# solonas13/REAL

Measured on AMD Instinct MI355X. Metric: aligned reads/sec (100 bp, k≤3) at 1/2/4/8 MI355X; achieved HBM GB/s vs peak, higher is better.
Workload: dtype u64

## Files before the change

### real_amd/csrc/match_kernel.hip

```cpp
#include "match_common.h"
#include "row_bytes.h"

#ifndef RH_ABLATE
#define RH_ABLATE 0
#endif
#ifndef RH_PHASE_TIMING
#define RH_PHASE_TIMING 0
#endif

#ifndef RH_PHASE_SUB
#define RH_PHASE_SUB 0
#endif
#if RH_PHASE_TIMING
#define PH_NOW() ((unsigned)__builtin_amdgcn_s_memrealtime())
#define PH_SUB(N, DT) do { if (RH_PHASE_SUB == (N)) s.tD += (DT); else if (RH_PHASE_SUB == 4) s.tD -= (DT); } while (0)
#else
#define PH_NOW() 0u
#endif
#define EB 8
#define MQ 16
#define QUEUE_BYTES (MQ * 64u * 5u + 6u * 64u * 4u)
enum : int { TK_STARTS = 0, TK_DIRECTORY = 1, TK_ROWS = 3, TK_ROWS_WIDE = 4 };
__host__ __device__ constexpr uint32_t stg_bytes(int W, int TK) { return TK >= TK_ROWS ? 11008u : (W <= 4 ? QUEUE_BYTES : 9728u); }
#define MQR 8u
static_assert(MQR == RH_QSPILL_SLOTS, "the spill area holds a second queue of MQR slots per lane");
#define NPEND2 24
#define MQR2 24u
#define STG_PAD 16u
#ifndef RH_KEEP_TW_MAXW
#define RH_KEEP_TW_MAXW 4
#endif
#define NPEND 4
#define SLOT_NONE 31u
#define SLOT_BIG 30u
#define PEND_OVF 0xffu
#define BIG_T 48u
#define BIG_T2 1024u

template <int W_, bool SCORES_, bool ALL_, int TK_, bool PASS2_>
struct LaneInst {
    static constexpr int W = W_;
    static constexpr bool SCORES = SCORES_;
    static constexpr bool ALL = ALL_;
    static constexpr int TK = TK_;
    static constexpr bool PASS2 = PASS2_;
    static constexpr bool DEFER = SCORES || ALL;
    static constexpr bool ROWS = TK >= TK_ROWS;
    static constexpr bool WIDE = TK == TK_ROWS_WIDE;
    static constexpr bool DIR = TK == TK_DIRECTORY;
    static constexpr bool HAS_PASS2 = ROWS && DEFER;
    static constexpr bool PAIRED = ROWS && !WIDE && DEFER && !PASS2;
    static constexpr int NP = PASS2 ? NPEND2 : NPEND;
    static constexpr uint32_t QSLOTS = PASS2 ? MQR2 : MQR;
    static constexpr uint32_t ROWBUF = QSLOTS * 64u * 5u, BKX = ROWBUF + 64u * 128u;
    static constexpr uint32_t BIG = PASS2 ? BIG_T2 : BIG_T;
    static constexpr uint32_t OVN = PASS2 ? 16u : 4u;
    static constexpr uint32_t STG = PASS2 ? BKX + 256u : stg_bytes(W, TK);
    static constexpr uint32_t STG_CAP = STG - STG_PAD - 32u;
    static_assert(!ROWS || (BKX + 256u <= STG && ROWBUF % 16 == 0), "row staging fits the wave's LDS region");
};
static_assert(QUEUE_BYTES % 16 == 0, "the staged bytes behind the queue are 16-byte aligned");

#define PM_LM_SHIFT 9
#define PM_LM_MASK (63u << PM_LM_SHIFT)
template <class T>
struct LaneState {
    static constexpr int W = T::W, NP = T::NP;
    uint64_t O[W];
    uint64_t shi, slo;
    uint32_t patl;
    int inv;
    __device__ __forceinline__ uint32_t nw() const { return (patl + 31) >> 5; }
    __device__ __forceinline__ uint64_t lastmask() const { return ~0ull << (64 - 2 * (patl - 32 * (nw() - 1))); }
    __device__ __forceinline__ uint32_t so(uint32_t l) const { return inv ? (patl - l) : 0u; }
    __device__ __forceinline__ float eps(double filter_mult) const { return (float)(filter_mult * (double)patl); }
    uint64_t r, o0, o1;
    uint64_t info;
    float iscore;
    uint32_t cpos, ck, cfrag;
    float cscore;
    bool cok;
    uint32_t crpos, ckk;
    uint32_t p_pos[NP], p_meta[NP];
    uint64_t p_tw[W <= RH_KEEP_TW_MAXW ? W : 1];
    uint32_t p_n, cslot;
    uint32_t nhit;
    unsigned cA, cB, cPw, cCw;
    __device__ __forceinline__ void addL(unsigned n) { cA += n; }
    __device__ __forceinline__ void addV(unsigned n) { cA += n << 4; }
    __device__ __forceinline__ void addS(unsigned n) { cA += n << 16; }
    __device__ __forceinline__ void addP(unsigned n) { if (T::PASS2) cPw += n; else cB += n; }
    __device__ __forceinline__ void addC(unsigned n) { if (T::PASS2) cCw += n; else cB += n << 11; }
    __device__ __forceinline__ unsigned getP() const { return T::PASS2 ? cPw : (cB & 2047u); }
    __device__ __forceinline__ unsigned getC() const { return T::PASS2 ? cCw : ((cB >> 11) & 2047u); }
    __device__ __forceinline__ void addH(unsigned n) { cB += n << 22; }
    __device__ __forceinline__ void reset_counters() { cA = cB = cPw = cCw = 0; }
    __device__ __forceinline__ void reset_read()
    {
        p_n = 0; cslot = SLOT_NONE;
#pragma unroll
        for (int j = 0; j < NP; ++j) { p_pos[j] = 0; p_meta[j] = 0; }
    }
    __device__ __forceinline__ void reset_strand(int inv_)
    {
        inv = inv_;
        cpos = 0xffffffffu; ck = 0; cfrag = 0; cscore = 1.0f; cok = false;
        crpos = 0xffffffffu; ckk = 0;
    }
#if RH_PHASE_TIMING
    unsigned tW, tD, tR;
#endif
};


template <int N>
__device__ __forceinline__ uint32_t sel(const uint32_t (&v)[N], uint32_t j)
{
    uint32_t r = 0;
#pragma unroll
    for (int i = 0; i < N; ++i) r |= j == (uint32_t)i ? v[i] : 0u;
    return r;
}
template <int N>
__device__ __forceinline__ float sel(const float (&v)[N], uint32_t j)
{
    uint32_t r = 0;
#pragma unroll
    for (int i = 0; i < N; ++i) r |= j == (uint32_t)i ? __float_as_uint(v[i]) : 0u;
    return __uint_as_float(r);
}
template <int N, class T>
__device__ __forceinline__ void put(T (&v)[N], uint32_t j, T x)
{
#pragma unroll
    for (int i = 0; i < N; ++i) v[i] = j == (uint32_t)i ? x : v[i];
}

template <class T>
__device__ __forceinline__ void deliver(const MatchArgs &a, LaneState<T> &s, uint32_t pos, uint32_t meta, float score)
{
    if (T::ALL) {
        unsigned long long slot = wave_append_slot(a.raw_count);
        if (slot < a.raw_cap) a.raw[slot] = make_uint4((uint32_t)s.r, pos, __float_as_uint(score), meta & ~PM_LM_MASK);
        s.nhit++;
    } else {
        fold_update<T::SCORES>((meta >> 8) & 1, a.t.fileid, pos, meta & 0xff, score, s.eps(a.filter_mult), meta >> 16, s.info, s.iscore);
    }
}

template <class T, class Row>
__device__ __forceinline__ void flush_pending(const MatchArgs &a, LaneState<T> &s, const double *sLL, const Row &qrow)
{
    constexpr int W = T::W, NP = T::NP;
    float sc[NP];
#pragma unroll
    for (int i = 0; i < NP; ++i) sc[i] = 1.0f;
#pragma unroll 1
    for (uint32_t j = 0; j < s.p_n; ++j) {
        if (!T::SCORES || (RH_ABLATE & 1)) break;
        const uint32_t pos = sel<NP>(s.p_pos, j);
        const uint32_t meta = sel<NP>(s.p_meta, j);
        const uint32_t inv = (meta >> 8) & 1;
        uint64_t Ow[W], tw[W];
        if ((int)inv == s.inv) {
#pragma unroll
            for (int i = 0; i < W; ++i) Ow[i] = s.O[i];
        } else {
            revcomp_words<W>(s.O, Ow, s.patl);
        }
        if (j == 0 && W <= RH_KEEP_TW_MAXW) {
#pragma unroll
            for (int i = 0; i < W; ++i) tw[i] = s.p_tw[W <= RH_KEEP_TW_MAXW ? i : 0];
        } else {
            const uint64_t wi = pos >> 5;
            const unsigned sh = 2u * (pos & 31);
            uint64_t t[W + 2];
#pragma unroll
            for (int i = 0; i <= W; i += 2) {
                U64x2 p2 = {0ull, 0ull};
                if ((uint32_t)i <= s.nw()) p2 = load2(a.t.text + wi + i);
                t[i] = p2.a; t[i + 1] = p2.b;
            }
#pragma unroll
            for (int i = 0; i < W; ++i) tw[i] = sh ? ((t[i] << sh) | (t[i + 1] >> (64 - sh))) : t[i];
        }
        const float v = score_location<W>(sLL, Ow, tw, s.patl, qrow, a.b.qual != nullptr, inv);
        put<NP>(sc, j, v);
    }
    auto lm_of = [&](uint32_t meta) { return (meta >> PM_LM_SHIFT) & 63u; };
    if (s.p_n == 1) {
        if (lm_of(s.p_meta[0])) deliver(a, s, s.p_pos[0], s.p_meta[0], sc[0]);
        return;
    }
    if (T::ALL) {
#pragma unroll 1
        for (uint32_t j = 0; j < s.p_n; ++j) {
            const uint32_t meta = sel<NP>(s.p_meta, j);
            if (lm_of(meta)) deliver(a, s, sel<NP>(s.p_pos, j), meta, sel<NP>(sc, j));
        }
        return;
    }
    if (s.p_n < 2) return;
    static_assert(NP <= 24, "two words of twelve ranks");
    uint64_t ord0 = 0, ord1 = 0;
    auto ord_at = [&](uint32_t rk) { return (uint32_t)((rk < 12 ? ord0 >> (5 * rk) : ord1 >> (5 * (rk - 12))) & 31u); };
#pragma unroll
    for (uint32_t j = 0; j < (uint32_t)NP; ++j) {
        const uint64_t kj = ((uint64_t)((s.p_meta[j] >> 8) & 1u) << 32) | s.p_pos[j];
        uint32_t rank = 0;
#pragma unroll
        for (uint32_t i = 0; i < (uint32_t)NP; ++i) {
            const uint64_t ki = ((uint64_t)((s.p_meta[i] >> 8) & 1u) << 32) | s.p_pos[i];
// ... 520 lines not shown
        }
        wave_lds_sync();
#if RH_PHASE_TIMING
        unsigned ph1 = PH_NOW();
        s.tW += ph1 - ph0;
#endif
        const bool mine = act && !(s.p_n == PEND_OVF) && !(RH_ABLATE & 8);
        const uint8_t *rowb = rowbuf + lane * 128;
        const uint32_t sw = lane & 7;
        auto row = [&](uint32_t d) { return *reinterpret_cast<const uint32_t *>(rowb + ((((d >> 2) ^ sw) << 4) | ((d & 3) << 2))); };
        uint32_t e_cnt = 0, e_j = 0, e_base = 0;
        bool e_ovf = false;
        uint32_t g, r;
        if (!wide) {
            g = rh_row_addr((uint32_t)la, sig_of(la), a.l, gbits).group;
            r = sig_of(5 - la) >> (a.l - pbits);
        } else {
            r = (uint32_t)(msig_wide(la) >> a.ix.fshift);
            g = r >> 28;
        }
        if (mine) {
            s.addL(1u);
            const uint32_t h0 = row(0), h1 = row(1);
            if (!rh_row_complex(h0, h1)) {
                e_cnt = ((g < 8 ? h0 : h1) >> (4 * (g & 7))) & 15u;
                const uint32_t m0 = g < 8 ? (g ? (h0 & (0xffffffffu >> (32 - 4 * g))) : 0u) : h0;
                const uint32_t m1 = g > 8 ? (h1 & (0xffffffffu >> (32 - 4 * (g - 8)))) : 0u;
                const uint32_t b0 = (m0 & 0x0f0f0f0fu) + ((m0 >> 4) & 0x0f0f0f0fu), b1 = (m1 & 0x0f0f0f0fu) + ((m1 >> 4) & 0x0f0f0f0fu);
                e_base = __builtin_amdgcn_sad_u8(b0, 0u, __builtin_amdgcn_sad_u8(b1, 0u, 0u));
            } else {
                e_ovf = true;
                uint32_t off = 0, sat255 = 0;
#pragma unroll
                for (int q = 0; q < 4; ++q) {
                    const uint32_t w = row(4 + q);
                    const int nb = (int)g - 4 * q;
                    const uint32_t below = nb <= 0 ? 0u : (nb >= 4 ? 0xffffffffu : ((1u << (8 * nb)) - 1u));
                    const uint32_t upto = nb < 0 ? 0u : (nb >= 3 ? 0xffffffffu : ((1u << (8 * (nb + 1))) - 1u));
                    off = __builtin_amdgcn_sad_u8(w & below, 0u, off);
                    if ((g >> 2) == (uint32_t)q) e_cnt = (w >> (8 * (g & 3))) & 255u;
                    const uint32_t y = ~w | ~upto;
                    sat255 |= (y - 0x01010101u) & ~y & 0x80808080u;
                }
                const bool sat = sat255 != 0;
                const uint32_t o0 = row(2), tot = row(3);
                e_base = o0 + off;
                if (sat) {
                    const uint2 kr = key_group_range(a.ix.ent[la], o0, o0 + tot, wide ? 28u : pbits, g);
                    e_base = kr.x; e_cnt = kr.y;
                }
            }
            if (!wide) s.addC(e_cnt);
            s.addP(e_cnt);
            if (e_cnt > T::BIG) { s.p_n = PEND_OVF; s.cslot = (!T::PASS2 && T::HAS_PASS2 && e_cnt <= BIG_T2) ? SLOT_NONE : SLOT_BIG; e_cnt = 0; }
            if (RH_ABLATE & 4) e_cnt = 0;
        }
        const uint32_t rk = wide ? rh_fp16(r) : (r >> (pbits - p16));
        U64x2 pre = {0ull, 0ull};
        if (e_ovf && e_cnt) pre = load2(reinterpret_cast<const uint64_t *>(a.ix.ent[la] + e_base));
        if (li + 1 < NL) ISSUE_ROWS(la + 1);
        auto take = [&](bool pass, uint32_t pos) {
            const bool merge = pass && qn && pos == q_last;
            if ((!wide || T::DEFER) && pass && !merge && qn >= 2) {
                for (uint32_t k = 0; k + 1 < qn; ++k)
                    if (q_pos[k * 64] == pos) { q_la[k * 64] |= (uint8_t)(1u << la); pass = false; break; }
            }
            if (pass && !merge && qn == T::QSLOTS) { s.p_n = PEND_OVF; e_cnt = 0; pass = false; }
            const uint32_t slot = merge ? qn - 1 : qn;
            const uint32_t lav = (merge ? q_lastla : 0u) | (1u << la);
            if (pass) { q_pos[slot * 64] = pos; q_la[slot * 64] = (uint8_t)lav; q_last = pos; q_lastla = lav; qn = slot + 1; }
        };
        auto passes = [&](uint32_t x) { return wide ? (x == 0u) : (__popc(((x >> 1) | x) & 0x55555555u) <= a.seedkmax); };
        uint32_t passm = 0;
        while (__any(!e_ovf && e_j < e_cnt)) {
#pragma unroll
            for (uint32_t u = 0; u < 4; ++u) {
                const uint32_t jj = e_j + u;
                const bool ok = !e_ovf && jj < e_cnt;
                const uint32_t h = ok ? rh_row_entry_hw(e_base + jj) : 4u;
                const uint32_t d0 = row(h >> 1);
                const uint32_t key = (h & 1) ? (d0 >> 16) : (d0 & 0xffffu);
                passm |= (ok && passes(key ^ rk) ? 1u : 0u) << (jj & 31u);
            }
            e_j += 4;
        }
        if (!T::PASS2 && T::HAS_PASS2 && __popc(passm) > NPEND) { s.p_n = PEND_OVF; passm = 0; e_cnt = 0; }
        while (__any(passm != 0)) {
            const bool step = passm != 0;
            const uint32_t jj = step ? (uint32_t)__ffs((int)passm) - 1u : 0u;
            passm &= passm - 1u;
            const uint32_t h = step ? rh_row_entry_hw(e_base + jj) : 4u;
            const uint32_t d0 = row(h >> 1), d1 = row((h >> 1) + 1);
            take(step, (h & 1) ? d1 : ((d0 >> 16) | (d1 << 16)));
        }
        auto take_ovf = [&](bool ok, uint2 e) { take(ok && passes(wide ? (e.x ^ r) : ((e.x & pmask) ^ r)), e.y); };
        if (__any(e_ovf && e_cnt)) {
            take_ovf(e_ovf && e_cnt > 0, make_uint2((uint32_t)pre.a, (uint32_t)(pre.a >> 32)));
            take_ovf(e_ovf && e_cnt > 1, make_uint2((uint32_t)pre.b, (uint32_t)(pre.b >> 32)));
        }
        e_j = 2;
        while (__any(e_ovf && e_j < e_cnt)) {
            uint2 e[T::OVN];
#pragma unroll
            for (uint32_t u = 0; u < T::OVN; ++u) e[u] = (e_ovf && e_j + u < e_cnt) ? a.ix.ent[la][e_base + e_j + u] : make_uint2(0u, 0u);
#pragma unroll
            for (uint32_t u = 0; u < T::OVN; ++u) take_ovf(e_ovf && e_j + u < e_cnt, e[u]);
            e_j += T::OVN;
        }
#if RH_PHASE_TIMING
        s.tD += PH_NOW() - ph1;
#endif
    }
    if (T::SCORES && qlast) ISSUE_QUALS();
#if RH_PHASE_TIMING
    const unsigned ph2 = PH_NOW();
#endif
    if (s.p_n == PEND_OVF) qn = 0;
    {
        CandText<T::W> c0;
        uint32_t rp0 = qn ? q_pos[0] : 0u;
        if (qn) cand_load(a, s, rp0, c0);
        for (uint32_t k = 0; k < qn; ++k) {
            CandText<T::W> c1;
            uint32_t rp1 = 0;
            if (k + 1 < qn) { rp1 = q_pos[(k + 1) * 64]; cand_load(a, s, rp1, c1); }
            process_loaded(a, s, sLL, rp0, (uint32_t)q_la[k * 64], c0);
            c0 = c1; rp0 = rp1;
        }
    }
#if RH_PHASE_TIMING
    s.tR += PH_NOW() - ph2;
#endif
    if (T::SCORES && qlast) ISSUE_QUALS_LATE();
#undef ISSUE_QUALS
#undef ISSUE_QUALS_LATE
#undef QUAL_DMA
}

template <class T>
__device__ __forceinline__ void match_rows_paired(const MatchArgs &a, LaneState<T> &s, const double *sLL, uint8_t *stg, bool act, uint32_t rhi,
                                                  uint32_t rlo)
{
    constexpr uint32_t QS = T::QSLOTS;
    uint32_t lane = threadIdx.x & 63;
    asm volatile("" : "+v"(lane));
    uint32_t *q_pos = reinterpret_cast<uint32_t *>(stg) + lane;
    uint8_t *q_la = stg + QS * 64 * 4 + lane;
    uint8_t *rowbuf = stg + T::ROWBUF;
    auto spill = [&](uint32_t k) -> uint2 & { return a.qspill[((size_t)(blockIdx.x * 4u + (threadIdx.x >> 6)) * QS + (k - QS)) * 64u + lane]; };
    const uint32_t bb = a.b_bits;
    const uint32_t gbits = a.ix.fbits, pbits = a.ix.pbits, p16 = pbits < 16 ? pbits : 16;
    const uint32_t pmask = (1u << pbits) - 1;
    const uint32_t mb = (1u << bb) - 1, fhi = (uint32_t)s.shi, flo = (uint32_t)s.slo;
    auto sig_of = [&](uint32_t strand, uint32_t la) {
        const uint32_t hi = strand ? rhi : fhi, lo = strand ? rlo : flo;
        const uint2 x = rh_list_segs(la);
        const uint32_t sa_ = ((x.x < 2 ? hi : lo) >> ((x.x & 1) ? 0u : bb)) & mb, sc_ = ((x.y < 2 ? hi : lo) >> ((x.y & 1) ? 0u : bb)) & mb;
        return (sa_ << bb) | sc_;
    };
    auto tbl_of = [](uint32_t li) { return li < 4 ? li >> 1 : li - 2; };
    struct Round { uint32_t row, g0, g1, s0; };
    auto round_of = [&](uint32_t li) -> Round {
        const uint32_t tbl = tbl_of(li), wbit = 1u << (gbits - 1);
        if (li < 4) {
            const RhRowAddr ra = rh_row_addr_pair(tbl, sig_of(li & 1u, tbl), a.l, gbits);
            return {ra.row, ra.group, ra.group | wbit, li & 1u};
        }
        const RhCanon c = rh_canon(sig_of(0u, tbl) >> bb, sig_of(1u, tbl) >> bb, bb);
        const RhRowAddr ra = rh_row_addr_canon(tbl, c, a.l, gbits);
        const uint32_t lo = c.self ? ra.group : ra.group & ~wbit;
        return {ra.row, lo, c.self ? lo : lo | wbit, c.which};
    };
    uint32_t qn = 0, qnf = 0, q_last = 0, q_lastla = 0;
    auto q_getp = [&](uint32_t k) { return k < QS ? q_pos[k * 64] : spill(k).x; };
    auto q_getl = [&](uint32_t k) { return k < QS ? (uint32_t)q_la[k * 64] : spill(k).y; };
    uint4 va0, va1, va2, va3, va4, va5, va6, va7;
    uint32_t *bkx = reinterpret_cast<uint32_t *>(stg + T::BKX);
#define ISSUE_ROWS_P(LI)                                                                                                    \
    do {                                                                                                                    \
        const Round rd_ = round_of(LI);                                                                                     \
        rnext = rd_.g0 | (rd_.g1 << 8) | (rd_.s0 << 16);                                                                    \
        bkx[(lane & 7) * 8 + (lane >> 3)] = act ? rd_.row : 0u;                                                             \
        __builtin_amdgcn_wave_barrier();                                                                                    \
        const uint4 b0_ = *reinterpret_cast<const uint4 *>(bkx + (lane >> 3) * 8);                                          \
        const uint4 b1_ = *reinterpret_cast<const uint4 *>(bkx + (lane >> 3) * 8 + 4);                                      \
        const uint4 *__restrict__ R_ = reinterpret_cast<const uint4 *>(a.ix.bkt[tbl_of(LI)]) + (lane & 7);                  \
        va0 = R_[(uint64_t)b0_.x * 8]; va1 = R_[(uint64_t)b0_.y * 8]; va2 = R_[(uint64_t)b0_.z * 8];                        \
        va3 = R_[(uint64_t)b0_.w * 8]; va4 = R_[(uint64_t)b1_.x * 8]; va5 = R_[(uint64_t)b1_.y * 8];                        \
        va6 = R_[(uint64_t)b1_.z * 8]; va7 = R_[(uint64_t)b1_.w * 8];                                                       \
    } while (0)
#define QUAL_DMA(SRC_OFF, LDS_ADDR, NBYTES, NCHUNK)                                                                                           \
    _Pragma("unroll") for (uint32_t i = 0; i < (NCHUNK); ++i)                                                                                 \
        if (16u * lane + 1024u * i + 16u <= (NBYTES)) {                                                                                       \
            const uint8_t *g_ = qsrc + (SRC_OFF) + 16u * lane + 1024u * i;                                                                    \
            uint32_t keep_;                                                                                                                   \
            asm volatile("s_mov_b32 %0, m0\n\ts_mov_b32 m0, %2\n\ts_nop 0\n\tglobal_load_lds_dwordx4 %1, off\n\ts_mov_b32 m0, %0"         \
                         : "=&s"(keep_) : "v"(g_), "s"((LDS_ADDR) + 1024u * i) : "memory");                                                   \
        }
    uint32_t rnext = 0;
    ISSUE_ROWS_P(0u);
#pragma unroll 1
    for (uint32_t li = 0; li < 6; ++li) {
        const uint32_t tbl = tbl_of(li);
        const bool pairt = li < 4;
#if RH_PHASE_TIMING
        const unsigned ph0 = PH_NOW();
#endif
        wave_lds_sync();
        {
            uint8_t *d = rowbuf + (lane >> 3) * 128 + (((lane & 7) ^ ((lane >> 3) & 7)) * 16);
            *reinterpret_cast<uint4 *>(d + 0 * 1024) = va0; *reinterpret_cast<uint4 *>(d + 1 * 1024) = va1;
            *reinterpret_cast<uint4 *>(d + 2 * 1024) = va2; *reinterpret_cast<uint4 *>(d + 3 * 1024) = va3;
            *reinterpret_cast<uint4 *>(d + 4 * 1024) = va4; *reinterpret_cast<uint4 *>(d + 5 * 1024) = va5;
            *reinterpret_cast<uint4 *>(d + 6 * 1024) = va6; *reinterpret_cast<uint4 *>(d + 7 * 1024) = va7;
        }
        wave_lds_sync();
#if RH_PHASE_TIMING
        unsigned ph1 = PH_NOW();
        s.tW += ph1 - ph0;
#endif
        const uint8_t *rowb = rowbuf + lane * 128;
        const uint32_t sw = lane & 7;
        auto row = [&](uint32_t d) { return *reinterpret_cast<const uint32_t *>(rowb + ((((d >> 2) ^ sw) << 4) | ((d & 3) << 2))); };
        auto row16 = [&](uint32_t B) { return (uint32_t)*reinterpret_cast<const uint16_t *>(rowb + rh_row_lds_byte(B, sw)); };
        const uint32_t g0 = rnext & 255u, g1 = (rnext >> 8) & 255u, s0 = rnext >> 16, la1 = pairt ? 5 - tbl : tbl;
        const uint32_t r0 = sig_of(s0, 5 - tbl) >> (a.l - pbits);
        const uint32_t r1 = sig_of(s0 ^ 1u, 5 - la1) >> (a.l - pbits);
        const bool mine = act && !(s.p_n == PEND_OVF) && !(RH_ABLATE & 8);
        const uint32_t h0 = row(0), h1 = row(1);
        const bool cplx = mine && rh_row_complex(h0, h1);
        uint32_t c0 = 0, c1 = 0, eb0 = 0, eb1 = 0;
        if (mine && !cplx) {
            const uint64_t hh = ((uint64_t)h1 << 32) | h0, ones = 0x1111111111111111ull;
            const uint64_t below0 = ones & ~(~0ull << (4 * g0));
            eb0 = nibble_dot(h0, (uint32_t)below0, nibble_dot(h1, (uint32_t)(below0 >> 32), 0u));
            c0 = (uint32_t)(hh >> (4 * g0)) & 15u;
            const uint64_t ext = (ones & ~(~0ull << (4 * g1))) ^ below0;
            eb1 = nibble_dot(h0, (uint32_t)ext, nibble_dot(h1, (uint32_t)(ext >> 32), eb0));
            c1 = (uint32_t)(hh >> (4 * g1)) & 15u;
            s.addL(2u);
            s.addC(c0 + c1);
            s.addP(c0 + c1);
            if (RH_ABLATE & 4) c0 = c1 = 0;
        }
        uint32_t e_cnt = 0;
        auto take = [&](bool pass, uint32_t pos, uint32_t strand, uint32_t la) {
            const bool merge = pass && qn && pos == q_last && (q_lastla >> 6) == strand;
            if (pass && !merge && qn >= 2) {
                for (uint32_t k = 0; k + 1 < qn; ++k)
                    if (q_getp(k) == pos && (q_getl(k) >> 6) == strand) {
                        if (k < QS) q_la[k * 64] |= (uint8_t)(1u << la); else spill(k).y |= 1u << la;
                        pass = false; break;
                    }
            }
            if (pass && !merge && (strand ? qn - qnf : qnf) == QS) { s.p_n = PEND_OVF; e_cnt = 0; pass = false; }
            const uint32_t slot = merge ? qn - 1 : qn;
            const uint32_t lav = (merge ? q_lastla : (strand << 6)) | (1u << la);
            if (pass) {
                if (slot < QS) { q_pos[slot * 64] = pos; q_la[slot * 64] = (uint8_t)lav; } else spill(slot) = make_uint2(pos, lav);
                q_last = pos; q_lastla = lav; qn = slot + 1;
                if (!merge && !strand) qnf++;
            }
        };
        auto passes = [&](uint32_t x) { return __popc(((x >> 1) | x) & 0x55555555u) <= a.seedkmax; };
        const uint32_t nhalf = __any(cplx) ? 2u : 1u;
#pragma unroll 1
        for (uint32_t half = 0; half < nhalf; ++half) {
            const uint32_t strand = s0 ^ half, la = half ? la1 : tbl;
            const uint32_t g = half ? g1 : g0, r = half ? r1 : r0;
            const bool e_ovf = cplx && !(s.p_n == PEND_OVF);
            uint32_t e_j = 0, e_base = 0;
            e_cnt = 0;
            if (e_ovf) {
                s.addL(1u);
                uint32_t off = 0, sat255 = 0;
#pragma unroll
                for (int q = 0; q < 4; ++q) {
                    const uint32_t w = row(4 + q);
                    const int nb = (int)g - 4 * q;
                    const uint32_t below = nb <= 0 ? 0u : (nb >= 4 ? 0xffffffffu : ((1u << (8 * nb)) - 1u));
                    const uint32_t upto = nb < 0 ? 0u : (nb >= 3 ? 0xffffffffu : ((1u << (8 * (nb + 1))) - 1u));
                    off = __builtin_amdgcn_sad_u8(w & below, 0u, off);
                    if ((g >> 2) == (uint32_t)q) e_cnt = (w >> (8 * (g & 3))) & 255u;
                    const uint32_t y = ~w | ~upto;
                    sat255 |= (y - 0x01010101u) & ~y & 0x80808080u;
                }
                const uint32_t o0 = row(2), tot = row(3);
                e_base = o0 + off;
                if (sat255 != 0) {
                    const uint2 kr = key_group_range(a.ix.ent[tbl], o0, o0 + tot, pbits, g);
                    e_base = kr.x; e_cnt = kr.y;
                }
                s.addC(e_cnt);
                s.addP(e_cnt);
                if (e_cnt > T::BIG) { s.p_n = PEND_OVF; s.cslot = e_cnt <= BIG_T2 ? SLOT_NONE : SLOT_BIG; e_cnt = 0; }
                if (RH_ABLATE & 4) e_cnt = 0;
            }
            U64x2 pre = {0ull, 0ull};
            if (e_ovf && e_cnt) pre = load2(reinterpret_cast<const uint64_t *>(a.ix.ent[tbl] + e_base));
            if (half == 0) {
                if (li + 1 < 6) ISSUE_ROWS_P(li + 1);
#if RH_PHASE_TIMING
                const unsigned ps1 = PH_NOW();
                PH_SUB(1, ps1 - ph1);
#endif
                static_assert(RH_ROW_CAP < 32 && 2 * 15 < 32, "one mask word for both groups of a simple row (one group taken twice: 2 x 15 entries)");
                const uint32_t ct = c0 + c1, d1 = eb1 - c0;
                uint32_t rk0 = r0 >> (pbits - p16), rk1 = r1 >> (pbits - p16);
                asm volatile("" : "+v"(rk0), "+v"(rk1));
                uint32_t passm = 0;
                while (__any(e_j < ct)) {
                    uint32_t key[4];
#pragma unroll
                    for (uint32_t u = 0; u < 4; ++u) {
                        const uint32_t jj = e_j + u;
                        const uint32_t ej = jj + (jj >= c0 ? d1 : eb0);
                        key[u] = row16(rh_row_key_byte(ej < RH_ROW_CAP - 1u ? ej : RH_ROW_CAP - 1u));
                    }
                    asm volatile("" : "+v"(key[0]), "+v"(key[1]), "+v"(key[2]), "+v"(key[3]));
#pragma unroll
                    for (uint32_t u = 0; u < 4; ++u) {
                        const uint32_t jj = e_j + u;
                        const uint32_t x = key[u] ^ (jj >= c0 ? rk1 : rk0);
                        passm |= ((jj < ct) & passes(x) ? 1u : 0u) << (jj & 31u);
                    }
                    e_j += 4;
                }
                const uint32_t low = (1u << c0) - 1u;
                if (__popc(passm & low) > NPEND || __popc(passm & ~low) > NPEND) { s.p_n = PEND_OVF; passm = 0; }
#if RH_PHASE_TIMING
                const unsigned ps2 = PH_NOW();
                PH_SUB(2, ps2 - ps1);
#endif
                while (__any(passm != 0)) {
                    const bool step = passm != 0;
                    const uint32_t jj = step ? (uint32_t)__ffs((int)passm) - 1u : 0u;
                    passm &= passm - 1u;
                    const bool sec = jj >= c0;
                    const uint32_t ej = step ? jj + (sec ? d1 : eb0) : 0u;
                    const uint32_t plo = row16(rh_row_pos_byte(ej, 0u)), phi = row16(rh_row_pos_byte(ej, 1u));
                    take(step, plo | (phi << 16), s0 ^ (sec ? 1u : 0u), sec ? la1 : tbl);
                }
#if RH_PHASE_TIMING
                PH_SUB(3, PH_NOW() - ps2);
#endif
            }
            auto take_ovf = [&](bool ok, uint2 e) { take(ok && passes((e.x & pmask) ^ r), e.y, strand, la); };
            if (__any(e_ovf && e_cnt)) {
                take_ovf(e_ovf && e_cnt > 0, make_uint2((uint32_t)pre.a, (uint32_t)(pre.a >> 32)));
                take_ovf(e_ovf && e_cnt > 1, make_uint2((uint32_t)pre.b, (uint32_t)(pre.b >> 32)));
            }
            e_j = 2;
            while (__any(e_ovf && e_j < e_cnt)) {
                uint2 e[T::OVN];
#pragma unroll
                for (uint32_t u = 0; u < T::OVN; ++u) e[u] = (e_ovf && e_j + u < e_cnt) ? a.ix.ent[tbl][e_base + e_j + u] : make_uint2(0u, 0u);
#pragma unroll
                for (uint32_t u = 0; u < T::OVN; ++u) take_ovf(e_ovf && e_j + u < e_cnt, e[u]);
                e_j += T::OVN;
            }
        }
#if RH_PHASE_TIMING
        if (RH_PHASE_SUB == 0 || RH_PHASE_SUB == 4) s.tD += PH_NOW() - ph1;
#endif
    }
    const uint32_t patl = act ? s.patl : 32u * T::W;
#pragma unroll 1
    for (uint32_t inv = 0; inv < 2; ++inv) {
        if (inv && act) {
            uint64_t R[T::W];
            revcomp_words<T::W>(s.O, R, patl);
#pragma unroll
            for (int j = 0; j < T::W; ++j) s.O[j] = R[j];
        }
        s.shi = inv ? rhi : fhi; s.slo = inv ? rlo : flo;
        s.reset_strand((int)inv);
        if (T::SCORES && inv) {
            const uint8_t *qsrc;
            uint32_t qbytes, qlate, qskew;
            if (quals_ahead<T>(a, s.o0, s.o1, qsrc, qbytes, qlate, qskew)) {
                wave_lds_sync();
                const uint32_t lds0 = __builtin_amdgcn_readfirstlane((uint32_t)(uintptr_t)(__attribute__((address_space(3))) uint8_t *)rowbuf);
                QUAL_DMA(qlate, lds0, qbytes - qlate, 9u)
                const uint32_t tail0 = qbytes & ~15u;
                if (lane < (qbytes & 15u)) rowbuf[tail0 - qlate + lane] = qsrc[tail0 + lane];
            }
        }
#if RH_PHASE_TIMING
        const unsigned ph2 = PH_NOW();
#endif
        if (s.p_n == PEND_OVF) qn = 0;
        auto next = [&](uint32_t k) { while (k < qn && (q_getl(k) >> 6) != inv) ++k; return k; };
        CandText<T::W> c0;
        uint32_t k = next(0u), rp0 = 0, la0 = 0;
        if (k < qn) { rp0 = q_getp(k); la0 = q_getl(k); cand_load(a, s, rp0, c0); }
        while (k < qn) {
            CandText<T::W> c1;
            const uint32_t k1 = next(k + 1);
            uint32_t rp1 = 0, la1 = 0;
            if (k1 < qn) { rp1 = q_getp(k1); la1 = q_getl(k1); cand_load(a, s, rp1, c1); }
            process_loaded(a, s, sLL, rp0, la0 & 63u, c0);
            c0 = c1; rp0 = rp1; la0 = la1; k = k1;
        }
#if RH_PHASE_TIMING
        s.tR += PH_NOW() - ph2;
#endif
    }
    if (T::SCORES) {
        const uint8_t *qsrc;
        uint32_t qbytes, qlate, qskew;
        if (quals_ahead<T>(a, s.o0, s.o1, qsrc, qbytes, qlate, qskew) && qlate) {
            wave_lds_sync();
            const uint32_t lds0 = __builtin_amdgcn_readfirstlane((uint32_t)(uintptr_t)(__attribute__((address_space(3))) uint8_t *)stg);
            QUAL_DMA(0u, lds0 + STG_PAD, qlate, 3u)
        }
    }
#undef QUAL_DMA
#undef ISSUE_ROWS_P
}

template <class T, int LA0, int LA1>
__device__ __forceinline__ void match_lists(const MatchArgs &a, LaneState<T> &s, const double *sLL, uint32_t *q_pos, uint8_t *q_la)
{
    if (T::DIR) { match_lists_directory<T, LA0, LA1>(a, s, sLL, q_pos, q_la); return; }
    uint32_t qn = 0;
    scan_lists<T, LA0, LA1>(a, s, q_pos, q_la, qn);
    for (uint32_t k = 0; k < qn && s.p_n != PEND_OVF; ++k)
        process_candidate(a, s, sLL, q_pos[k * 64], (uint32_t)q_la[k * 64]);
}

template <class T>
__device__ __forceinline__ void match_read(const MatchArgs &a, LaneState<T> &s, const double *sLL, uint8_t *stg, uint32_t *q_pos, uint8_t *q_la,
                                           bool act)
{
    const uint32_t patl = act ? s.patl : 32u * T::W;
    s.reset_read();
    uint64_t rhi = 0, rlo = 0;
    if (act) seed_halves<T::W>(s.O, a.l, s.shi, s.slo, rhi, rlo);
    else { s.shi = s.slo = 0; }
    if constexpr (T::PAIRED) { match_rows_paired<T>(a, s, sLL, stg, act, (uint32_t)rhi, (uint32_t)rlo); return; }
    for (int inv = 0; inv < 2; ++inv) {
        if constexpr (!T::ROWS) {
            if (s.p_n == PEND_OVF) break;
        }
        if (inv && act) {
            uint64_t R[T::W];
            revcomp_words<T::W>(s.O, R, patl);
#pragma unroll
            for (int j = 0; j < T::W; ++j) s.O[j] = R[j];
            s.shi = rhi; s.slo = rlo;
        }
        s.reset_strand(inv);
        const bool go = !T::ROWS || (act && !(s.p_n == PEND_OVF));
        if (!T::ALL && !T::SCORES) {
            if constexpr (T::ROWS) match_lists_rows<T, 0, 1>(a, s, sLL, stg, go, false);
            else match_lists<T, 0, 1>(a, s, sLL, q_pos, q_la);
            const unsigned st = (unsigned)(s.info >> ST_SHIFT), er = (unsigned)(s.info >> ER_SHIFT) & 15;
            if constexpr (T::ROWS) match_lists_rows<T, 1, 6>(a, s, sLL, stg, go && !(st == (unsigned)(inv ? ST_REVERSE : ST_STRAIGHT) && er == 0), false);
            else if (!(st == (unsigned)(inv ? ST_REVERSE : ST_STRAIGHT) && er == 0)) match_lists<T, 1, 6>(a, s, sLL, q_pos, q_la);
        } else if constexpr (T::ROWS) {
            match_lists_rows<T, 0, 6>(a, s, sLL, stg, go, !T::PASS2 && inv != 0);
        } else {
            match_lists<T, 0, 6>(a, s, sLL, q_pos, q_la);
        }
    }
}

template <int W, bool SCORES, bool ALL, int TK, bool PASS2>
__global__ __launch_bounds__(256) __attribute__((amdgpu_waves_per_eu(PASS2 ? 2 : (W <= 5 ? 3 : 2)))) void match_kernel(MatchArgs a_)
{
    using T = LaneInst<W, SCORES, ALL, TK, PASS2>;
    constexpr uint32_t STG = T::STG;
    static_assert(!PASS2 || T::HAS_PASS2, "the second pass exists for bucket rows with parked hits only");
    __shared__ double sLL[SCORES ? RH_LL_SLOTS : 1];
    __shared__ __attribute__((aligned(16))) uint8_t smem[4 * STG];
    if (SCORES) {
        for (int i = threadIdx.x; i < 1024; i += 256) sLL[i] = a_.LL[i];
        if (threadIdx.x == 0) sLL[RH_LL_ZERO] = 0.0;
        __syncthreads();
    }
    const uint64_t n_items = PASS2 ? (uint64_t)*a_.ovf_count : a_.b.n_reads;
    const uint64_t n_tiles = (n_items + 63) / 64;
    uint32_t *const tile_ctr = PASS2 ? a_.tile_ctr2 : a_.tile_ctr;
    uint32_t next_raw = 0;
    if ((threadIdx.x & 63) == 0) next_raw = atomicAdd(tile_ctr, 1u);
    while (true) {
    const uint64_t tile = (uint32_t)__builtin_amdgcn_readfirstlane((int)next_raw);
    if (tile >= n_tiles) break;
    if ((threadIdx.x & 63) == 0) next_raw = atomicAdd(tile_ctr, 1u);
    uint32_t tid = threadIdx.x;
    asm volatile("" : "+v"(tid));
    const __attribute__((address_space(4))) MatchArgs *pa = (const __attribute__((address_space(4))) MatchArgs *)__builtin_amdgcn_kernarg_segment_ptr();
    asm volatile("" : "+s"(pa));
    const MatchArgs &a = *(const MatchArgs *)pa;
    const uint32_t lane = tid & 63;
    uint8_t *stg = smem + (tid >> 6) * STG;
    uint32_t *q_pos = reinterpret_cast<uint32_t *>(stg) + lane;
    uint8_t *q_la = stg + MQ * 64 * 4 + lane;
    const unsigned ph_start = PH_NOW();
    LaneState<T> s;
    s.reset_counters();
#if RH_PHASE_TIMING
    s.tW = s.tD = s.tR = 0;
    unsigned tQ = 0, tS = 0;
#endif
    s.info = 0; s.iscore = 0.f; s.o0 = s.o1 = 0;
    unsigned cR = 0;
    const uint64_t n = a.b.n_reads;

    const uint64_t item = tile * 64 + lane;
    const bool have = item < n_items;
    const uint64_t r = PASS2 ? (have ? (uint64_t)a.ovf_list[item] : n) : item;
// ... 189 lines not shown
```

Before: 4.569 billion.

## Defer complex-row overflow groups into a wave-cooperative flat walk

Lanes holding complex rows no longer walk their overflow entry groups one lane at a time. They record descriptors (base, count, table, list, strand) in a per-wave LDS list across all six list rounds. In the last round the wave builds prefix sums and spreads the entries over all 64 lanes, then routes passing hits back to the owning lane through an LDS atomicMin slot and shuffles. This is meant to remove the lane divergence and serial gathers caused by a few heavy lanes, at the cost of extra LDS, wave syncs and a per-hit routing loop, with an in-place fallback when the descriptor list fills.

```diff
diff --git a/real_amd/csrc/complex_walk.h b/real_amd/csrc/complex_walk.h
--- /dev/null
+++ b/real_amd/csrc/complex_walk.h
@@ -0,0 +1,64 @@
+#pragma once
+#include <stdint.h>
+#if defined(__HIPCC__)
+#define RH_HD __host__ __device__
+#else
+#define RH_HD
+#endif
+
+#define CW_MAX_DESC 64u
+#define CW_NONE 0xffffffffu
+static inline RH_HD uint32_t cw_pack(uint32_t lane, uint32_t cnt, uint32_t table, uint32_t list, uint32_t strand)
+{
+    return lane | ((cnt - 1u) << 6) | (table << 12) | (list << 14) | (strand << 17);
+}
+static inline RH_HD uint32_t cw_lane(uint32_t m) { return m & 63u; }
+static inline RH_HD uint32_t cw_cnt(uint32_t m) { return ((m >> 6) & 63u) + 1u; }
+static inline RH_HD uint32_t cw_table(uint32_t m) { return (m >> 12) & 3u; }
+static inline RH_HD uint32_t cw_list(uint32_t m) { return (m >> 14) & 7u; }
+static inline RH_HD uint32_t cw_strand(uint32_t m) { return (m >> 17) & 1u; }
+
+static inline RH_HD uint32_t cw_byte_sum(uint32_t x, uint32_t acc)
+{
+#if defined(__HIP_DEVICE_COMPILE__)
+    return __builtin_amdgcn_sad_u8(x, 0u, acc);
+#else
+    return acc + (x & 255u) + ((x >> 8) & 255u) + ((x >> 16) & 255u) + (x >> 24);
+#endif
+}
+
+struct CwGroup { uint32_t off, cnt, sat; };
+static inline RH_HD void cw_header_word(uint32_t w, int nb, CwGroup &o)
+{
+    const uint32_t below = nb <= 0 ? 0u : (nb >= 4 ? 0xffffffffu : ((1u << (8 * nb)) - 1u));
+    const uint32_t upto = nb < 0 ? 0u : (nb >= 3 ? 0xffffffffu : ((1u << (8 * (nb + 1))) - 1u));
+    o.off = cw_byte_sum(w & below, o.off);
+    if (nb >= 0 && nb < 4) o.cnt = (w >> (8 * nb)) & 255u;
+    const uint32_t y = ~w | ~upto;
+    o.sat |= (y - 0x01010101u) & ~y & 0x80808080u;
+}
+static inline RH_HD void cw_header2(const uint32_t (&w)[4], uint32_t g0, uint32_t g1, CwGroup &a, CwGroup &b)
+{
+    a.off = a.cnt = a.sat = 0u;
+    b.off = b.cnt = b.sat = 0u;
+#if defined(__HIP_DEVICE_COMPILE__)
+#pragma unroll
+#endif
+    for (int q = 0; q < 4; ++q) {
+        cw_header_word(w[q], (int)g0 - 4 * q, a);
+        cw_header_word(w[q], (int)g1 - 4 * q, b);
+    }
+}
+
+static inline RH_HD uint32_t cw_flat_find(const uint32_t *pre, uint32_t n, uint32_t t)
+{
+    uint32_t d = 0;
+#if defined(__HIP_DEVICE_COMPILE__)
+#pragma unroll
+#endif
+    for (uint32_t step = CW_MAX_DESC / 2u; step; step >>= 1) {
+        const uint32_t c = d + step;
+        if (c < n && pre[c] <= t) d = c;
+    }
+    return d;
+}
diff --git a/real_amd/csrc/match_kernel.hip b/real_amd/csrc/match_kernel.hip
--- a/real_amd/csrc/match_kernel.hip
+++ b/real_amd/csrc/match_kernel.hip
@@ -1,5 +1,6 @@
 #include "match_common.h"
 #include "row_bytes.h"
+#include "complex_walk.h"
 
 #ifndef RH_ABLATE
 #define RH_ABLATE 0
@@ -55,9 +56,11 @@
     static constexpr uint32_t ROWBUF = QSLOTS * 64u * 5u, BKX = ROWBUF + 64u * 128u;
     static constexpr uint32_t BIG = PASS2 ? BIG_T2 : BIG_T;
     static constexpr uint32_t OVN = PASS2 ? 16u : 4u;
-    static constexpr uint32_t STG = PASS2 ? BKX + 256u : stg_bytes(W, TK);
-    static constexpr uint32_t STG_CAP = STG - STG_PAD - 32u;
+    static constexpr uint32_t CWCAP = 44u, CWLIST = stg_bytes(W, TK), CWBYTES = PAIRED ? CWCAP * 8u : 0u;
+    static constexpr uint32_t STG = PASS2 ? BKX + 256u : stg_bytes(W, TK) + CWBYTES;
+    static constexpr uint32_t STG_CAP = STG - CWBYTES - STG_PAD - 32u;
     static_assert(!ROWS || (BKX + 256u <= STG && ROWBUF % 16 == 0), "row staging fits the wave's LDS region");
+    static_assert(CWCAP <= CW_MAX_DESC && CWBYTES % 16 == 0, "one descriptor per lane builds the prefix sums; the regions stay 16-byte aligned");
 };
 static_assert(QUEUE_BYTES % 16 == 0, "the staged bytes behind the queue are 16-byte aligned");
 
@@ -884,12 +887,12 @@
     const uint32_t gbits = a.ix.fbits, pbits = a.ix.pbits, p16 = pbits < 16 ? pbits : 16;
     const uint32_t pmask = (1u << pbits) - 1;
     const uint32_t mb = (1u << bb) - 1, fhi = (uint32_t)s.shi, flo = (uint32_t)s.slo;
-    auto sig_of = [&](uint32_t strand, uint32_t la) {
-        const uint32_t hi = strand ? rhi : fhi, lo = strand ? rlo : flo;
+    auto sig_from = [&](uint32_t hi, uint32_t lo, uint32_t la) {
         const uint2 x = rh_list_segs(la);
         const uint32_t sa_ = ((x.x < 2 ? hi : lo) >> ((x.x & 1) ? 0u : bb)) & mb, sc_ = ((x.y < 2 ? hi : lo) >> ((x.y & 1) ? 0u : bb)) & mb;
         return (sa_ << bb) | sc_;
     };
+    auto sig_of = [&](uint32_t strand, uint32_t la) { return sig_from(strand ? rhi : fhi, strand ? rlo : flo, la); };
     auto tbl_of = [](uint32_t li) { return li < 4 ? li >> 1 : li - 2; };
     struct Round { uint32_t row, g0, g1, s0; };
     auto round_of = [&](uint32_t li) -> Round {
@@ -930,6 +933,28 @@
                          : "=&s"(keep_) : "v"(g_), "s"((LDS_ADDR) + 1024u * i) : "memory");                                                   \
         }
     uint32_t rnext = 0;
+    uint32_t e_cnt = 0;
+    auto take = [&](bool pass, uint32_t pos, uint32_t strand, uint32_t la) {
+        const bool merge = pass && qn && pos == q_last && (q_lastla >> 6) == strand;
+        if (pass && !merge && qn >= 2) {
+            for (uint32_t k = 0; k + 1 < qn; ++k)
+                if (q_getp(k) == pos && (q_getl(k) >> 6) == strand) {
+                    if (k < QS) q_la[k * 64] |= (uint8_t)(1u << la); else spill(k).y |= 1u << la;
+                    pass = false; break;
+                }
+        }
+        if (pass && !merge && (strand ? qn - qnf : qnf) == QS) { s.p_n = PEND_OVF; e_cnt = 0; pass = false; }
+        const uint32_t slot = merge ? qn - 1 : qn;
+        const uint32_t lav = (merge ? q_lastla : (strand << 6)) | (1u << la);
+        if (pass) {
+            if (slot < QS) { q_pos[slot * 64] = pos; q_la[slot * 64] = (uint8_t)lav; } else spill(slot) = make_uint2(pos, lav);
+            q_last = pos; q_lastla = lav; qn = slot + 1;
+            if (!merge && !strand) qnf++;
+        }
+    };
+    auto passes = [&](uint32_t x) { return __popc(((x >> 1) | x) & 0x55555555u) <= a.seedkmax; };
+    uint2 *cwl = reinterpret_cast<uint2 *>(stg + T::CWLIST);
+    uint32_t cw_n = 0;
     ISSUE_ROWS_P(0u);
 #pragma unroll 1
     for (uint32_t li = 0; li < 6; ++li) {
@@ -975,121 +1000,183 @@
             s.addP(c0 + c1);
             if (RH_ABLATE & 4) c0 = c1 = 0;
         }
-        uint32_t e_cnt = 0;
-        auto take = [&](bool pass, uint32_t pos, uint32_t strand, uint32_t la) {
-            const bool merge = pass && qn && pos == q_last && (q_lastla >> 6) == strand;
-            if (pass && !merge && qn >= 2) {
-                for (uint32_t k = 0; k + 1 < qn; ++k)
-                    if (q_getp(k) == pos && (q_getl(k) >> 6) == strand) {
-                        if (k < QS) q_la[k * 64] |= (uint8_t)(1u << la); else spill(k).y |= 1u << la;
-                        pass = false; break;
+        uint32_t xb0 = 0, xc0 = 0, xb1 = 0, xc1 = 0;
+        bool inplace = false;
+        if (__any(cplx)) {
+            if (cplx) {
+                const uint32_t w[4] = {row(4), row(5), row(6), row(7)};
+                const uint32_t o0 = row(2), tot = row(3);
+                CwGroup ga, gb;
+                cw_header2(w, g0, g1, ga, gb);
+                s.addL(1u);
+                xb0 = o0 + ga.off; xc0 = ga.cnt;
+                if (ga.sat) {
+                    const uint2 kr = key_group_range(a.ix.ent[tbl], o0, o0 + tot, pbits, g0);
+                    xb0 = kr.x; xc0 = kr.y;
+                }
+                s.addC(xc0);
+                s.addP(xc0);
+                if (xc0 > T::BIG) { s.p_n = PEND_OVF; s.cslot = xc0 <= BIG_T2 ? SLOT_NONE : SLOT_BIG; xc0 = 0; }
+                else {
+                    s.addL(1u);
+                    xb1 = o0 + gb.off; xc1 = gb.cnt;
+                    if (gb.sat) {
+                        const uint2 kr = key_group_range(a.ix.ent[tbl], o0, o0 + tot, pbits, g1);
+                        xb1 = kr.x; xc1 = kr.y;
                     }
-            }
-            if (pass && !merge && (strand ? qn - qnf : qnf) == QS) { s.p_n = PEND_OVF; e_cnt = 0; pass = false; }
-            const uint32_t slot = merge ? qn - 1 : qn;
-            const uint32_t lav = (merge ? q_lastla : (strand << 6)) | (1u << la);
-            if (pass) {
-                if (slot < QS) { q_pos[slot * 64] = pos; q_la[slot * 64] = (uint8_t)lav; } else spill(slot) = make_uint2(pos, lav);
-                q_last = pos; q_lastla = lav; qn = slot + 1;
-                if (!merge && !strand) qnf++;
-            }
+                    s.addC(xc1);
+                    s.addP(xc1);
+                    if (xc1 > T::BIG) { s.p_n = PEND_OVF; s.cslot = xc1 <= BIG_T2 ? SLOT_NONE : SLOT_BIG; xc0 = xc1 = 0; }
+                }
+                if (RH_ABLATE & 4) xc0 = xc1 = 0;
+            }
+            const uint64_t m0 = __ballot(xc0 != 0), m1 = __ballot(xc1 != 0);
+            const uint32_t n0 = (uint32_t)__popcll(m0), n1 = (uint32_t)__popcll(m1);
+            inplace = cw_n + n0 + n1 > T::CWCAP;
+            if (!inplace) {
+                const uint32_t i0 = cw_n + __builtin_amdgcn_mbcnt_hi((uint32_t)(m0 >> 32), __builtin_amdgcn_mbcnt_lo((uint32_t)m0, 0u));
+                const uint32_t i1 = cw_n + n0 + __builtin_amdgcn_mbcnt_hi((uint32_t)(m1 >> 32), __builtin_amdgcn_mbcnt_lo((uint32_t)m1, 0u));
+                if (xc0) cwl[i0] = make_uint2(xb0, cw_pack(lane, xc0, tbl, tbl, s0));
+                if (xc1) cwl[i1] = make_uint2(xb1, cw_pack(lane, xc1, tbl, la1, s0 ^ 1u));
+                cw_n += n0 + n1;
+                xc0 = xc1 = 0;
+            }
+        }
+        const bool walk = li == 5 && cw_n != 0;
+        uint32_t *cw_pre = bkx;
+        uint32_t cw_total = 0;
+        auto fetch = [&](uint32_t t, uint2 &e, uint32_t &m, uint32_t &k) {
+            const bool ok = t < cw_total;
+            const uint32_t d = cw_flat_find(cw_pre, cw_n, ok ? t : 0u);
+            const uint2 ds = cwl[d];
+            const uint32_t tb = cw_table(ds.y), own = cw_lane(ds.y), st = cw_strand(ds.y);
+            const uint2 *E = tb == 0u ? a.ix.ent[0] : tb == 1u ? a.ix.ent[1] : tb == 2u ? a.ix.ent[2] : a.ix.ent[3];
+            e = make_uint2(0u, 0u);
+            if (ok) e = E[ds.x + (t - cw_pre[d])];
+            m = ok ? ds.y : CW_NONE;
+            const uint32_t ohf = __shfl(fhi, (int)own), olf = __shfl(flo, (int)own), ohr = __shfl(rhi, (int)own), olr = __shfl(rlo, (int)own);
+            k = sig_from(st ? ohr : ohf, st ? olr : olf, 5u - cw_list(ds.y)) >> (a.l - pbits);
         };
-        auto passes = [&](uint32_t x) { return __popc(((x >> 1) | x) & 0x55555555u) <= a.seedkmax; };
-        const uint32_t nhalf = __any(cplx) ? 2u : 1u;
+        uint2 e_c = make_uint2(0u, 0u), e_n = make_uint2(0u, 0u);
+        uint32_t m_c = CW_NONE, k_c = 0, m_n = CW_NONE, k_n = 0;
+#if RH_PHASE_TIMING
+        const unsigned pw0 = PH_NOW();
+#endif
+        if (walk) {
+            static_assert(T::CWCAP * 4u <= 256u, "the prefix sums lie in the place of the bucket numbers");
+            wave_lds_sync();
+            const uint32_t cnt = lane < cw_n ? cw_cnt(cwl[lane].y) : 0u;
+            uint32_t inc = cnt;
+#pragma unroll
+            for (uint32_t d = 1; d < 64; d <<= 1) {
+                const uint32_t v = __shfl_up(inc, d);
+                if (lane >= d) inc += v;
+            }
+            cw_total = __builtin_amdgcn_readlane(inc, 63);
+            wave_lds_sync();
+            if (lane < cw_n) cw_pre[lane] = inc - cnt;
+            wave_lds_sync();
+            fetch(lane, e_c, m_c, k_c);
+            if (cw_total > 64u) fetch(64u + lane, e_n, m_n, k_n);
+        }
+#if RH_PHASE_TIMING
+        const unsigned pw1 = PH_NOW();
+#endif
+        U64x2 pre = {0ull, 0ull};
+        if (inplace && xc0) pre = load2(reinterpret_cast<const uint64_t *>(a.ix.ent[tbl] + xb0));
+        if (li + 1 < 6) ISSUE_ROWS_P(li + 1);
+#if RH_PHASE_TIMING
+        const unsigned ps1 = PH_NOW();
+        PH_SUB(1, (ps1 - ph1) - (pw1 - pw0));
+#endif
+        {
+            static_assert(RH_ROW_CAP < 32 && 2 * 15 < 32, "one mask word for both groups of a simple row (one group taken twice: 2 x 15 entries)");
+            const uint32_t ct = c0 + c1, d1 = eb1 - c0;
+            uint32_t rk0 = r0 >> (pbits - p16), rk1 = r1 >> (pbits - p16);
+            asm volatile("" : "+v"(rk0), "+v"(rk1));
+            uint32_t passm = 0, e_j = 0;
+            while (__any(e_j < ct)) {
+                uint32_t key[4];
+#pragma unroll
+                for (uint32_t u = 0; u < 4; ++u) {
+                    const uint32_t jj = e_j + u;
+                    const uint32_t ej = jj + (jj >= c0 ? d1 : eb0);
+                    key[u] = row16(rh_row_key_byte(ej < RH_ROW_CAP - 1u ? ej : RH_ROW_CAP - 1u));
+                }
+                asm volatile("" : "+v"(key[0]), "+v"(key[1]), "+v"(key[2]), "+v"(key[3]));
+#pragma unroll
+                for (uint32_t u = 0; u < 4; ++u) {
+                    const uint32_t jj = e_j + u;
+                    const uint32_t x = key[u] ^ (jj >= c0 ? rk1 : rk0);
+                    passm |= ((jj < ct) & passes(x) ? 1u : 0u) << (jj & 31u);
+                }
+                e_j += 4;
+            }
+            const uint32_t low = (1u << c0) - 1u;
+            if (__popc(passm & low) > NPEND || __popc(passm & ~low) > NPEND) { s.p_n = PEND_OVF; passm = 0; }
+#if RH_PHASE_TIMING
+            const unsigned ps2 = PH_NOW();
+            PH_SUB(2, ps2 - ps1);
+#endif
+            while (__any(passm != 0)) {
+                const bool step = passm != 0;
+                const uint32_t jj = step ? (uint32_t)__ffs((int)passm) - 1u : 0u;
+                passm &= passm - 1u;
+                const bool sec = jj >= c0;
+                const uint32_t ej = step ? jj + (sec ? d1 : eb0) : 0u;
+                const uint32_t plo = row16(rh_row_pos_byte(ej, 0u)), phi = row16(rh_row_pos_byte(ej, 1u));
+                take(step, plo | (phi << 16), s0 ^ (sec ? 1u : 0u), sec ? la1 : tbl);
+            }
+#if RH_PHASE_TIMING
+            PH_SUB(3, PH_NOW() - ps2);
+#endif
+        }
+        if (inplace) {
 #pragma unroll 1
-        for (uint32_t half = 0; half < nhalf; ++half) {
-            const uint32_t strand = s0 ^ half, la = half ? la1 : tbl;
-            const uint32_t g = half ? g1 : g0, r = half ? r1 : r0;
-            const bool e_ovf = cplx && !(s.p_n == PEND_OVF);
-            uint32_t e_j = 0, e_base = 0;
-            e_cnt = 0;
-            if (e_ovf) {
-                s.addL(1u);
-                uint32_t off = 0, sat255 = 0;
-#pragma unroll
-                for (int q = 0; q < 4; ++q) {
-                    const uint32_t w = row(4 + q);
-                    const int nb = (int)g - 4 * q;
-                    const uint32_t below = nb <= 0 ? 0u : (nb >= 4 ? 0xffffffffu : ((1u << (8 * nb)) - 1u));
-                    const uint32_t upto = nb < 0 ? 0u : (nb >= 3 ? 0xffffffffu : ((1u << (8 * (nb + 1))) - 1u));
-                    off = __builtin_amdgcn_sad_u8(w & below, 0u, off);
-                    if ((g >> 2) == (uint32_t)q) e_cnt = (w >> (8 * (g & 3))) & 255u;
-                    const uint32_t y = ~w | ~upto;
-                    sat255 |= (y - 0x01010101u) & ~y & 0x80808080u;
-                }
-                const uint32_t o0 = row(2), tot = row(3);
-                e_base = o0 + off;
-                if (sat255 != 0) {
-                    const uint2 kr = key_group_range(a.ix.ent[tbl], o0, o0 + tot, pbits, g);
-                    e_base = kr.x; e_cnt = kr.y;
-                }
-                s.addC(e_cnt);
-                s.addP(e_cnt);
-                if (e_cnt > T::BIG) { s.p_n = PEND_OVF; s.cslot = e_cnt <= BIG_T2 ? SLOT_NONE : SLOT_BIG; e_cnt = 0; }
-                if (RH_ABLATE & 4) e_cnt = 0;
-            }
-            U64x2 pre = {0ull, 0ull};
-            if (e_ovf && e_cnt) pre = load2(reinterpret_cast<const uint64_t *>(a.ix.ent[tbl] + e_base));
-            if (half == 0) {
-                if (li + 1 < 6) ISSUE_ROWS_P(li + 1);
-#if RH_PHASE_TIMING
-                const unsigned ps1 = PH_NOW();
-                PH_SUB(1, ps1 - ph1);
-#endif
-                static_assert(RH_ROW_CAP < 32 && 2 * 15 < 32, "one mask word for both groups of a simple row (one group taken twice: 2 x 15 entries)");
-                const uint32_t ct = c0 + c1, d1 = eb1 - c0;
-                uint32_t rk0 = r0 >> (pbits - p16), rk1 = r1 >> (pbits - p16);
-                asm volatile("" : "+v"(rk0), "+v"(rk1));
-                uint32_t passm = 0;
-                while (__any(e_j < ct)) {
-                    uint32_t key[4];
-#pragma unroll
-                    for (uint32_t u = 0; u < 4; ++u) {
-                        const uint32_t jj = e_j + u;
-                        const uint32_t ej = jj + (jj >= c0 ? d1 : eb0);
-                        key[u] = row16(rh_row_key_byte(ej < RH_ROW_CAP - 1u ? ej : RH_ROW_CAP - 1u));
-                    }
-                    asm volatile("" : "+v"(key[0]), "+v"(key[1]), "+v"(key[2]), "+v"(key[3]));
-#pragma unroll
-                    for (uint32_t u = 0; u < 4; ++u) {
-                        const uint32_t jj = e_j + u;
-                        const uint32_t x = key[u] ^ (jj >= c0 ? rk1 : rk0);
-                        passm |= ((jj < ct) & passes(x) ? 1u : 0u) << (jj & 31u);
-                    }
-                    e_j += 4;
-                }
-                const uint32_t low = (1u << c0) - 1u;
-                if (__popc(passm & low) > NPEND || __popc(passm & ~low) > NPEND) { s.p_n = PEND_OVF; passm = 0; }
-#if RH_PHASE_TIMING
-                const unsigned ps2 = PH_NOW();
-                PH_SUB(2, ps2 - ps1);
-#endif
-                while (__any(passm != 0)) {
-                    const bool step = passm != 0;
-                    const uint32_t jj = step ? (uint32_t)__ffs((int)passm) - 1u : 0u;
-                    passm &= passm - 1u;
-                    const bool sec = jj >= c0;
-                    const uint32_t ej = step ? jj + (sec ? d1 : eb0) : 0u;
-                    const uint32_t plo = row16(rh_row_pos_byte(ej, 0u)), phi = row16(rh_row_pos_byte(ej, 1u));
-                    take(step, plo | (phi << 16), s0 ^ (sec ? 1u : 0u), sec ? la1 : tbl);
-                }
-#if RH_PHASE_TIMING
-                PH_SUB(3, PH_NOW() - ps2);
-#endif
-            }
-            auto take_ovf = [&](bool ok, uint2 e) { take(ok && passes((e.x & pmask) ^ r), e.y, strand, la); };
-            if (__any(e_ovf && e_cnt)) {
-                take_ovf(e_ovf && e_cnt > 0, make_uint2((uint32_t)pre.a, (uint32_t)(pre.a >> 32)));
-                take_ovf(e_ovf && e_cnt > 1, make_uint2((uint32_t)pre.b, (uint32_t)(pre.b >> 32)));
-            }
-            e_j = 2;
-            while (__any(e_ovf && e_j < e_cnt)) {
-                uint2 e[T::OVN];
-#pragma unroll
-                for (uint32_t u = 0; u < T::OVN; ++u) e[u] = (e_ovf && e_j + u < e_cnt) ? a.ix.ent[tbl][e_base + e_j + u] : make_uint2(0u, 0u);
-#pragma unroll
-                for (uint32_t u = 0; u < T::OVN; ++u) take_ovf(e_ovf && e_j + u < e_cnt, e[u]);
-                e_j += T::OVN;
+            for (uint32_t half = 0; half < 2; ++half) {
+                const uint32_t strand = s0 ^ half, la = half ? la1 : tbl, r = half ? r1 : r0;
+                const uint32_t e_base = half ? xb1 : xb0;
+                e_cnt = s.p_n == PEND_OVF ? 0u : (half ? xc1 : xc0);
+                const bool e_ovf = e_cnt != 0;
+                if (half) pre = e_ovf ? load2(reinterpret_cast<const uint64_t *>(a.ix.ent[tbl] + e_base)) : U64x2{0ull, 0ull};
+                auto take_ovf = [&](bool ok, uint2 e) { take(ok && passes((e.x & pmask) ^ r), e.y, strand, la); };
+                if (__any(e_ovf)) {
+                    take_ovf(e_cnt > 0, make_uint2((uint32_t)pre.a, (uint32_t)(pre.a >> 32)));
+                    take_ovf(e_cnt > 1, make_uint2((uint32_t)pre.b, (uint32_t)(pre.b >> 32)));
+                }
+                uint32_t e_j = 2;
+                while (__any(e_j < e_cnt)) {
+                    uint2 e[T::OVN];
+#pragma unroll
+                    for (uint32_t u = 0; u < T::OVN; ++u) e[u] = (e_j + u < e_cnt) ? a.ix.ent[tbl][e_base + e_j + u] : make_uint2(0u, 0u);
+#pragma unroll
+                    for (uint32_t u = 0; u < T::OVN; ++u) take_ovf(e_j + u < e_cnt, e[u]);
+                    e_j += T::OVN;
+                }
+            }
+        }
+        if (walk) {
+            uint32_t *cw_slot = reinterpret_cast<uint32_t *>(rowbuf);
+#pragma unroll 1
+            for (uint32_t t0 = 0; t0 < cw_total; t0 += 64u) {
+                bool pend = m_c != CW_NONE && passes((e_c.x & pmask) ^ k_c);
+                const uint32_t own = cw_lane(m_c);
+                while (__any(pend)) {
+                    wave_lds_sync();
+                    cw_slot[lane] = CW_NONE;
+                    wave_lds_sync();
+                    if (pend) atomicMin(cw_slot + own, lane);
+                    wave_lds_sync();
+                    const uint32_t from = cw_slot[lane];
+                    const bool hit = from != CW_NONE;
+                    const int src = (int)(hit ? from : lane);
+                    const uint32_t pos = __shfl(e_c.y, src), tag = __shfl(m_c, src);
+                    if (pend && cw_slot[own] == lane) pend = false;
+                    take(hit, pos, cw_strand(tag), cw_list(tag));
+                }
+                e_c = e_n; m_c = m_n; k_c = k_n;
+                m_n = CW_NONE;
+                if (t0 + 128u < cw_total) fetch(t0 + 128u + lane, e_n, m_n, k_n);
             }
         }
 #if RH_PHASE_TIMING
```

Result: faster. 4.636 billion (median of 6 runs) (+1.5%).
